# ZwwWayne/mmMOT

Hardware: NVIDIA H100
Metric: frame-pairs/sec at N=128 dets (higher is better)
Workload: dtype f32 (tensor-core engine: FP16 hi/lo split operands, fp32 accumulate)

## Files before the change

include/mmmot_b200.h:

```cpp
#ifndef MMMOT_B200_H
#define MMMOT_B200_H

#include <stddef.h>
#include <stdint.h>

#ifdef __cplusplus
extern "C" {
#endif

#define MMMOT_ABI_VERSION 2

enum {
  MMMOT_E_ARG = -1,
  MMMOT_E_WORKSPACE = -2,
  MMMOT_E_SHAPE = -3,
  MMMOT_E_RANGE = -4
};

enum { MMMOT_FUSION_A = 0, MMMOT_FUSION_B = 1, MMMOT_FUSION_C = 2 };
enum { MMMOT_AFF_MULTIPLY = 0, MMMOT_AFF_MINUS_ABS = 1, MMMOT_AFF_MINUS = 2 };
enum { MMMOT_SM_NONE = 0, MMMOT_SM_SINGLE = 1, MMMOT_SM_DUAL = 2, MMMOT_SM_DUAL_ADD = 3, MMMOT_SM_DUAL_MAX = 4 };
enum { MMMOT_END_AVG = 0, MMMOT_END_MAX = 1 };

enum mmmot_weight_id {
// ... 100 lines not shown
                     const double* det_planes, const int* det_frame, int n_dets, int* split, void* workspace,
                     size_t workspace_bytes, void* stream);
int mmmot_prep_scatter(const float* points, const int* frame_offsets, int n_frames, int stride,
                       const double* fov_planes, const double* det_planes, const int* det_frame, int n_dets,
                       const int* split, int out_channels, float* out_points, void* workspace,
                       size_t workspace_bytes, void* stream);

int mmmot_crop_resize_max_taps(void);
size_t mmmot_crop_resize_workspace(int n_det, long total_rows, int out_size, int taps);
int mmmot_crop_resize(const unsigned char* image, int img_h, int img_w, const int* boxes, const long long* row_off,
                      int n_det, long total_rows, int max_crop_h, int out_size, int taps, const float* mean_std,
                      float* out, void* workspace, size_t workspace_bytes, void* stream);

int mmmot_set_engine(int engine);

int mmmot_set_kseg(int chunks);

int mmmot_set_debug(int flags);

int mmmot_debug_linear(const float* Wt, const void* Wp, float wp_scale, const float* bias, const float* X,
                       float* Y, int M, int K, int S, int engine, void* stream);

int mmmot_debug_simt(int mode, int M, int K, const float* Wt, const float* bias, int relu, const float* X, long x_gs,
                     long x_ks, const float* sc, const float* sh, int S, int groups, const void* tile_tab, int num_tiles,
                     float* Y, long y_gs, long y_ms, void* part, void* stream);

int mmmot_debug_simt_op(int mode, int M, int K, const float* Wt, const float* bias, int relu, const float* X, long x_gs,
                        long x_ks, const float* sc, const float* sh, int n, int m, int Lf, int H, int W, int Cin, int S,
                        int groups, const void* tile_tab, int num_tiles, const float* addend, const int* seg, int ld_add,
                        float* Y, long y_gs, long y_ms, void* part, void* stream);

int mmmot_debug_gen_prefetch(int gen, int m);
int mmmot_debug_gen_staged(int gen, int m);
int mmmot_debug_gen(int gen, int M, int K, const void* Wp, float wp_scale, const float* bias, int relu, const float* src,
                    int ld_src, const float* gsc, const float* gsh, int n, int m, int Lf, int S, int groups, long x_gs,
                    long y_gs, const void* tile_tab, int num_tiles, float* Y, long y_ms, void* part, int* prefetched,
                    void* stream);

int mmmot_debug_pn_contraction(const int* det_split, const int* h_det_split, int pairs, int L, long max_tiles, void* tiles,
                               int* cnt, int* gstart, int* seg, void* ctab, long* n_tiles, const void* Wp, float wp_scale,
                               const float* bias, int M, int K, const void* Xhi, float* Y, void* part, const float* addend,
                               int ld_add, unsigned long long* segsum, const float* sc, const float* sh, void* stream);

int mmmot_debug_pn_stats(const int* det_split, const int* h_det_split, int pairs, int L, const void* Xhi, int K,
                         const float* Wt, const void* Wp, float wp_scale, const float* bias, int M, const float* addend,
                         const float* gamma, const float* beta, float* sc, float* sh, double* stats, double* mom,
                         unsigned long long* detsum, void* workspace, size_t workspace_bytes, void* stream);

int mmmot_debug_linear_planar(const void* Wp, float wp_scale, const float* bias, const void* Xhi, float* Y,
                              int M, int K, long rows, void* stream);
int mmmot_debug_conv_planar(const void* Wp, float wp_scale, const float* bias, const void* Xhi, void* Yhi,
                            int n_img, int H, int W, int C, int M, float* kseg_scratch ,
                            void* stream);

int mmmot_debug_conv_plan(int n_img, int H, int W, int C, int M, int want_pool, int use_kseg, int* plan);
int mmmot_debug_conv_layer(const void* Wp, const void* Wpx, float wp_scale, const float* bias, const void* Xhi, long x_plane,
                           int n_img, int H, int W, int C, int M, void* Yhi, long y_plane, long y_plane_pooled,
                           int* did_pool, unsigned long long* pool_sum, float* kseg_scratch, int* status, int* plan,
                           void* stream);
int mmmot_debug_vgg_conv0(const float* crops, int n_img, int H, int W, const float* wt, const float* bias, const void* Wp,
                          float wp_scale, const void* Wpx, void* Yhi, long y_plane, void* cols, int* status, int* variant,
                          void* stream);

int mmmot_debug_stage_layout(int stage, int pairs, int n, int m, size_t* offsets, int* tensor_cores);
int mmmot_debug_skip_heads(const mmmot_weights* wts, const float* pooled0, const float* pooled1, const float* pooled2,
                           const float* pooled3, int n_img, int L, float* feats, void* stream);
// ... 14 lines not shown
```

mmmot_b200/_lib.py:

```python
import ctypes
import os
import re

_HERE = os.path.dirname(os.path.abspath(__file__))
LIB_PATH = os.path.join(_HERE, "libmmmot_sm90a.so")
HEADER_PATH = os.path.join(os.path.dirname(_HERE), "include", "mmmot_b200.h")

ABI_VERSION = 2
SCORE_SIGMOID, SCORE_THRESHOLD = 1, 2
FUSION = {"A": 0, "B": 1, "C": 2}
AFFINITY = {"multiply": 0, "minus_abs": 1, "minus": 2}
SOFTMAX = {"none": 0, "single": 1, "dual": 2, "dual_add": 3, "dual_max": 4}
END_MODE = {"avg": 0, "max": 1}

W = dict(
    VGG_WT0=0, VGG_B0=13, SKIP0=26, PN_L1=66, PN_WHAT=86, PN_WHGT=87, PN_BH=88, PN_GHW=89, PN_GHB=90,
    PN_WOT=91, PN_BO=92, PN_GOW=93, PN_GOB=94,
    FU_WPT=95, FU_BP=96, FU_GPW=97, FU_GPB=98, FU_WIT=99, FU_BI=100, FU_GIW=101, FU_GIB=102,
    FU_GATE_PT=103, FU_GATE_PB=104, FU_GATE_IT=105, FU_GATE_IB=106,
    WD_W1T=107, WD_B1=108, WD_W2T=109, WD_B2=110, WD_W3=111, WD_B3=112,
    AF_W01T=113, AF_B01=114, AF_G1W=115, AF_G1B=116, AF_G0W=117, AF_G0B=118,
    AF_W2T=119, AF_B2=120, AF_G2W=121, AF_G2B=122, AF_W3T=123, AF_B3=124, AF_G3W=125, AF_G3B=126,
    AF_W4=127, AF_B4=128,
    NE_W1T=129, NE_B1=130, NE_G1W=131, NE_G1B=132, NE_W2T=133, NE_B2=134, NE_G2W=135, NE_G2B=136,
# ... 11 lines not shown
class MmmotError(RuntimeError):
    pass


_vp, _i, _l, _f, _sz = ctypes.c_void_p, ctypes.c_int, ctypes.c_long, ctypes.c_float, ctypes.c_size_t
_wp = ctypes.POINTER(Weights)

SIGNATURES = {
    "mmmot_abi_version": (_i, []),
    "mmmot_device_info": (_i, [ctypes.POINTER(_i)] * 3),
    "mmmot_launch_count": (ctypes.c_ulonglong, []),
    "mmmot_set_engine": (_i, [_i]),
    "mmmot_set_debug": (_i, [_i]),
    "mmmot_set_kseg": (_i, [_i]),
    "mmmot_debug_linear": (_i, [_vp, _vp, _f, _vp, _vp, _vp, _i, _i, _i, _i, _vp]),
    "mmmot_debug_simt": (_i, [_i, _i, _i, _vp, _vp, _i, _vp, _l, _l, _vp, _vp, _i, _i, _vp, _i, _vp, _l, _l, _vp, _vp]),
    "mmmot_debug_simt_op": (_i, [_i, _i, _i, _vp, _vp, _i, _vp, _l, _l, _vp, _vp, _i, _i, _i, _i, _i, _i, _i, _i, _vp, _i,
                                 _vp, _vp, _i, _vp, _l, _l, _vp, _vp]),
    "mmmot_debug_linear_planar": (_i, [_vp, _f, _vp, _vp, _vp, _i, _i, _l, _vp]),
    "mmmot_debug_conv_planar": (_i, [_vp, _f, _vp, _vp, _vp, _i, _i, _i, _i, _i, _vp, _vp]),
    "mmmot_debug_conv_plan": (_i, [_i, _i, _i, _i, _i, _i, _i, ctypes.POINTER(_i)]),
    "mmmot_debug_conv_layer": (_i, [_vp, _vp, _f, _vp, _vp, _l, _i, _i, _i, _i, _i, _vp, _l, _l, ctypes.POINTER(_i), _vp, _vp,
                                    _vp, ctypes.POINTER(_i), _vp]),
    "mmmot_debug_vgg_conv0": (_i, [_vp, _i, _i, _i, _vp, _vp, _vp, _f, _vp, _vp, _l, _vp, _vp, ctypes.POINTER(_i), _vp]),
    "mmmot_timing_enable": (_i, [_i]),
    "mmmot_timing_tag_count": (_i, []),
    "mmmot_timing_tag_name": (ctypes.c_char_p, [_i]),
    "mmmot_timing_collect_tags": (_i, [ctypes.POINTER(ctypes.c_double)] * 3 + [ctypes.POINTER(ctypes.c_long)]),
    "mmmot_status_reset": (_i, [_vp, _vp]),
    "mmmot_status_check": (_i, [_vp, _vp]),
    "mmmot_fetch_pinned_i32": (_i, [_vp, _vp, _l, _vp]),
    "mmmot_debug_gen_prefetch": (_i, [_i, _i]),
    "mmmot_debug_gen_staged": (_i, [_i, _i]),
    "mmmot_debug_gen": (_i, [_i, _i, _i, _vp, _f, _vp, _i, _vp, _i, _vp, _vp, _i, _i, _i, _i, _i, _l, _l, _vp, _i, _vp, _l, _vp,
                             ctypes.POINTER(_i), _vp]),
    "mmmot_debug_pn_contraction": (_i, [_vp, _vp, _i, _i, _l, _vp, _vp, _vp, _vp, _vp, ctypes.POINTER(_l), _vp, _f, _vp, _i, _i,
                                        _vp, _vp, _vp, _vp, _i, _vp, _vp, _vp, _vp]),
    "mmmot_debug_pn_stats": (_i, [_vp, _vp, _i, _i, _vp, _i, _vp, _vp, _f, _vp, _i, _vp, _vp, _vp, _vp, _vp, _vp, _vp, _vp, _vp,
                                  _sz, _vp]),
    "mmmot_debug_stage_layout": (_i, [_i, _i, _i, _i, ctypes.POINTER(_sz), ctypes.POINTER(_i)]),
    "mmmot_debug_skip_heads": (_i, [_wp, _vp, _vp, _vp, _vp, _i, _i, _vp, _vp]),
    "mmmot_timing_collect": (_i, [ctypes.POINTER(ctypes.c_double), ctypes.POINTER(ctypes.c_double), ctypes.POINTER(ctypes.c_long)]),
    "mmmot_appearance_workspace": (_sz, [_i, _i, _i]),
    "mmmot_appearance_fwd": (_i, [_wp, _vp, _i, _i, _i, _i, _vp, _vp, _sz, _vp]),
    "mmmot_appearance_train_workspace": (_sz, [_i, _i, _i]),
    "mmmot_appearance_train_fwd": (_i, [_wp, _vp, _i, _i, _i, _i, _vp, _vp, _vp, _vp, _vp, _sz, _vp]),
    "mmmot_pointnet_train_workspace": (_sz, [_i, _i, _l]),
    "mmmot_pointnet_train_fwd": (_i, [_wp, _vp, _vp, _vp, _i, _i, _vp, _vp, _vp, _sz, _vp]),
    "mmmot_w_det_train_workspace": (_sz, [_i]),
    "mmmot_w_det_train_fwd": (_i, [_wp, _i, _vp, _vp, _vp, _vp, _sz, _vp]),
    "mmmot_pointnet_workspace": (_sz, [_i, _i, _l]),
    "mmmot_pointnet_fwd": (_i, [_wp, _vp, _vp, _vp, _i, _i, _vp, _vp, _sz, _vp]),
    "mmmot_fusion_det_workspace": (_sz, [_i, _i]),
    "mmmot_fusion_det_fwd": (_i, [_wp, _i, _i, _f, _i, _i, _vp, _vp, _vp, _sz, _vp]),
    "mmmot_affinity_workspace": (_sz, [_i, _i, _i]),
    "mmmot_affinity_fwd": (_i, [_wp, _i, _i, _i, _i, _i, _i, _vp, _vp, _vp, _vp, _vp, _sz, _vp]),
    "mmmot_crop_workspace": (_sz, [_i, _i]),
    "mmmot_crop_count": (_i, [_vp, _i, _i, _vp, _i, _i, _vp, _vp, _sz, _vp]),
    "mmmot_crop_scatter": (_i, [_vp, _i, _i, _vp, _i, _i, _vp, _i, _vp, _vp, _sz, _vp]),
    "mmmot_prep_workspace": (_sz, [_i, _i, _i]),
    "mmmot_prep_count": (_i, [_vp, _vp, _i, _i, _vp, _vp, _vp, _i, _vp, _vp, _sz, _vp]),
    "mmmot_prep_scatter": (_i, [_vp, _vp, _i, _i, _vp, _vp, _vp, _i, _vp, _i, _vp, _vp, _sz, _vp]),
    "mmmot_crop_resize_max_taps": (_i, []),
    "mmmot_crop_resize_workspace": (_sz, [_i, _l, _i, _i]),
    "mmmot_crop_resize": (_i, [_vp, _i, _i, _vp, _vp, _i, _l, _i, _i, _i, _vp, _vp, _vp, _sz, _vp]),
    "mmmot_lp_workspace": (_sz, [_i, _i, _i]),
# ... 40 lines not shown
```

mmmot_b200/csrc/api.cu:

```cuda
#include <algorithm>
#include <atomic>

#include "common.cuh"

static std::atomic<unsigned long long> g_launches{0};

void mm_count_launch() { g_launches.fetch_add(1, std::memory_order_relaxed); }

extern "C" unsigned long long mmmot_launch_count(void) { return g_launches.load(); }

extern "C" int mmmot_abi_version(void) { return MMMOT_ABI_VERSION; }

int mm_sm_count(int* sms) {
  static std::atomic<int> cache[64];
  int dev = 0;
  MM_CUDA(cudaGetDevice(&dev));
  int v = cache[dev & 63].load(std::memory_order_relaxed);
  if (!v) {
    MM_CUDA(cudaDeviceGetAttribute(&v, cudaDevAttrMultiProcessorCount, dev));
    cache[dev & 63].store(v, std::memory_order_relaxed);
  }
  *sms = v;
  return 0;
}
// ... 202 lines not shown
  p.Wt = Wt; p.ldw = M; p.bias = bias; p.M = M; p.K = K; p.relu = relu;
  if (tile_tab) {
    p.tile_tab = (const int4*)tile_tab; p.num_tiles = num_tiles;
  } else {
    p.S = S; p.tiles_per_group = mm_cdiv(S, 128); p.num_tiles = p.tiles_per_group * groups;
  }
  p.X = X; p.x_gs = x_gs; p.x_ks = x_ks; p.sc = sc; p.sh = sh;
  p.n = n; p.m = m; p.Lf = Lf;
  p.H = H; p.W = W; p.Cin = Cin;
  p.addend = addend; p.seg = seg; p.ld_add = ld_add;
  p.Y = Y; p.y_gs = y_gs; p.y_ms = y_ms;
  p.part = (double2*)part;
  cudaStream_t st = (cudaStream_t)stream;
  switch (mode) {
    case XM_DIRECT: return gemm_simt_launch<XM_DIRECT>(p, st);
    case XM_NORM_RELU: return gemm_simt_launch<XM_NORM_RELU>(p, st);
    case XM_PAIR_MUL: return gemm_simt_launch<XM_PAIR_MUL>(p, st);
    case XM_PAIR_ABS: return gemm_simt_launch<XM_PAIR_ABS>(p, st);
    case XM_PAIR_SUB: return gemm_simt_launch<XM_PAIR_SUB>(p, st);
    default: return gemm_simt_launch<XM_CONV3>(p, st);
  }
}

extern "C" int mmmot_debug_gen_prefetch(int gen, int m) {
  if (gen < gen::GEN_PAIR_MUL || gen > gen::GEN_COPY) return MMMOT_E_ARG;
  return gen_prefetch(gen, m, mm_debug_flags()) ? 1 : 0;
}

extern "C" int mmmot_debug_gen_staged(int gen, int m) {
  if (gen < gen::GEN_PAIR_MUL || gen > gen::GEN_COPY) return MMMOT_E_ARG;
  return gen_staged(gen, m, mm_debug_flags()) ? 1 : 0;
}

extern "C" int mmmot_debug_gen(int gen, int M, int K, const void* Wp, float wp_scale, const float* bias, int relu,
                               const float* src, int ld_src, const float* gsc, const float* gsh, int n, int m, int Lf, int S,
                               int groups, long x_gs, long y_gs, const void* tile_tab, int num_tiles, float* Y, long y_ms,
                               void* part, int* prefetched, void* stream) {
  if (M <= 0 || K <= 0) return MMMOT_E_ARG;
  GemmP p = gemm_defaults();
  p.bias = bias; p.M = M; p.K = K; p.relu = relu;
  if (tile_tab) {
    if (num_tiles <= 0) return MMMOT_E_ARG;
    p.tile_tab = (const int4*)tile_tab; p.num_tiles = num_tiles;
  } else {
    if (S <= 0 || groups <= 0) return MMMOT_E_ARG;
    p.S = S; p.tiles_per_group = mm_cdiv(S, tc::BN); p.num_tiles = p.tiles_per_group * groups;
    p.x_gs = x_gs; p.y_gs = y_gs;
  }
  p.Y = Y; p.y_ms = y_ms;
  p.part = (double2*)part;
  const uint4* w = (const uint4*)Wp;
  cudaStream_t st = (cudaStream_t)stream;
  switch (gen) {
    case gen::GEN_PAIR_MUL: return gemm_gen_launch<gen::GEN_PAIR_MUL>(p, w, wp_scale, src, ld_src, gsc, gsh, n, m, Lf, st, prefetched);
    case gen::GEN_PAIR_ABS: return gemm_gen_launch<gen::GEN_PAIR_ABS>(p, w, wp_scale, src, ld_src, gsc, gsh, n, m, Lf, st, prefetched);
    case gen::GEN_PAIR_SUB: return gemm_gen_launch<gen::GEN_PAIR_SUB>(p, w, wp_scale, src, ld_src, gsc, gsh, n, m, Lf, st, prefetched);
    case gen::GEN_NORM: return gemm_gen_launch<gen::GEN_NORM>(p, w, wp_scale, src, ld_src, gsc, gsh, n, m, Lf, st, prefetched);
    case gen::GEN_COPY: return gemm_gen_launch<gen::GEN_COPY>(p, w, wp_scale, src, ld_src, gsc, gsh, n, m, Lf, st, prefetched);
    default: return MMMOT_E_ARG;
  }
}

extern "C" int mmmot_debug_linear_planar(const void* Wp, float wp_scale, const float* bias, const void* Xhi,
                                         float* Y, int M, int K, long rows, void* stream) {
  if (!Wp || !Xhi || !Y || M <= 0 || K <= 0 || rows <= 0) return MMMOT_E_ARG;
  GemmP p = gemm_defaults();
// ... 53 lines not shown
```

mmmot_b200/csrc/gemm_gen.cuh:

```cuda
#pragma once
#include "gemm_tma.cuh"

namespace gen {

using namespace tc;

enum { GEN_PAIR_MUL = 0, GEN_PAIR_ABS = 1, GEN_PAIR_SUB = 2, GEN_NORM = 3, GEN_COPY = 4 };

constexpr int G_EPI_WARPS = 8, G_PROD_WARP0 = 8, G_PROD_WARPS = 8;
constexpr int G_THREADS = (G_PROD_WARP0 + G_PROD_WARPS) * 32;
constexpr int G_CONS_REGS = 176, G_PROD_REGS = 80;
static_assert(256 * G_CONS_REGS + 256 * G_PROD_REGS <= launch_regs(G_THREADS) * G_THREADS, "register split exceeds the CTA's pool");
constexpr int G_DET_BYTES = 128 * BK * 4, G_OBJ_BYTES = 2 * BK * 4;
static_assert(G_DET_BYTES == A_SUB && A_SUB % 1024 == 0, "the detection box fills the stage's free 1024-aligned slot");
constexpr int G_SRC_AHEAD = STAGES - 1;
constexpr size_t G_SMEM_BYTES = (size_t)STAGES * STAGE_BYTES + 1024 + 256 + STAGES * G_OBJ_BYTES;
constexpr int G_MAX_K = 512;
__host__ __device__ constexpr bool staged(int GEN, bool PAIRED) { return PAIRED && GEN <= GEN_PAIR_SUB; }

struct GenP {
  TcP t;
  const float* src;
  int ld_src;
  const float* gsc;
  const float* gsh;
  int n, m, Lf;
};

__device__ __forceinline__ void lds128(uint32_t addr, float4& v) {
  asm volatile("ld.shared.v4.f32 {%0, %1, %2, %3}, [%4];" : "=f"(v.x), "=f"(v.y), "=f"(v.z), "=f"(v.w) : "r"(addr));
}
__device__ __forceinline__ void ld_global_256(const float* p, float (&v)[8]) {
  asm volatile("ld.global.nc.v4.f32 {%0, %1, %2, %3}, [%8];\n\tld.global.nc.v4.f32 {%4, %5, %6, %7}, [%8+16];"
               : "=f"(v[0]), "=f"(v[1]), "=f"(v[2]), "=f"(v[3]), "=f"(v[4]), "=f"(v[5]), "=f"(v[6]), "=f"(v[7])
               : "l"(p));
}

template <int GEN, bool PAIRED>
static __global__ void __launch_bounds__(G_THREADS, 1)
gemm_gen_kernel(const GenP P, const __grid_constant__ CUtensorMap map_det, const __grid_constant__ CUtensorMap map_obj) {
  const GemmP& p = P.t.g;
  extern __shared__ uint8_t smem_raw[];
  __shared__ __align__(16) float s_gsc[GEN == GEN_NORM ? G_MAX_K : 4], s_gsh[GEN == GEN_NORM ? G_MAX_K : 4];
  const uint32_t raw = smem_u32(smem_raw);
  const uint32_t base = (raw + 1023u) & ~1023u;
  uint8_t* sm = smem_raw + (base - raw);
  const uint32_t bar0 = base + STAGES * STAGE_BYTES;
  auto full_bar = [&](int s) { return bar0 + 8u * s; };
  auto empty_bar = [&](int s) { return bar0 + 8u * (STAGES + s); };
  const uint32_t free_bar = bar0 + 8u * (2 * STAGES);
  auto src_full = [&](int s) { return bar0 + 8u * (2 * STAGES + 1 + s); };
  auto src_empty = [&](int s) { return bar0 + 8u * (3 * STAGES + 1 + s); };
  const uint32_t obj0 = bar0 + 256;
  float* img = reinterpret_cast<float*>(sm);

  const int tid = threadIdx.x, warp = tid >> 5, lane = tid & 31;
  const int mgroups = P.t.m_tiles;
  const long total_tiles = (long)p.num_tiles * mgroups;
  const int KC = P.t.k_chunks;

  if (tid == 0) {
    for (int s = 0; s < STAGES; s++) {
      mbar_init(full_bar(s), 1 + G_PROD_WARPS);
      mbar_init(empty_bar(s), G_EPI_WARPS);
      if (staged(GEN, PAIRED)) {
        mbar_init(src_full(s), 1);
        mbar_init(src_empty(s), G_PROD_WARPS);
      }
    }
    mbar_init(free_bar, G_EPI_WARPS);
    asm volatile("fence.mbarrier_init.release.cluster;" ::: "memory");
  }
  __syncthreads();

  auto tile_cols = [&](int nt, int& g, int& c0, int& len) {
    if (p.tile_tab) { const int4 tt = p.tile_tab[nt]; g = tt.x; c0 = tt.y; len = tt.z; return; }
    g = nt / p.tiles_per_group;
    c0 = (nt - g * p.tiles_per_group) * BN;
    len = min(BN, p.S - c0);
  };

  if (warp < G_EPI_WARPS) {
    asm volatile("setmaxnreg.inc.sync.aligned.u32 %0;" ::"n"(G_CONS_REGS));
    const int q = warp & 3, half = warp >> 2;
    uint32_t it = 0;
    float acc[2][64];
    auto clear_acc = [&]() {
#pragma unroll
      for (int mb = 0; mb < 2; mb++)
#pragma unroll
        for (int i = 0; i < 64; i++) acc[mb][i] = 0.f;
    };
    if (!staged(GEN, PAIRED)) clear_acc();
    for (long t = blockIdx.x; t < total_tiles; t += gridDim.x) {
      const int mg = (int)(t % mgroups);
      const int nt = (int)(t / mgroups);
      int g, c0, len;
      tile_cols(nt, g, c0, len);
      if (staged(GEN, PAIRED)) clear_acc();
      for (int kc = 0; kc < KC; kc++, it++) {
        const int s = it % STAGES;
        mbar_wait(full_bar(s), (it / STAGES) & 1);
        const uint32_t sa = base + s * STAGE_BYTES, sb = sa + 2 * A_SUB + half * (128 / 8) * 128;
        if (!(P.t.dbg & 8)) {
          wgmma_fence();
#pragma unroll
          for (int ks = 0; ks < 2; ks++) {
            const uint64_t b_hi = smem_desc(sb + ks * 2 * B_LBO, B_LBO, SBO);
            const uint64_t b_lo = smem_desc(sb + B_HALF + ks * 2 * B_LBO, B_LBO, SBO);
#pragma unroll
            for (int mb = 0; mb < 2; mb++) {
              const uint32_t a = sa + mb * 8 * SBO + ks * 2 * A_LBO;
              const uint64_t a_hi = smem_desc(a, A_LBO, SBO), a_lo = smem_desc(a + A_HALF, A_LBO, SBO);
              wgmma_n128(acc[mb], a_hi, b_hi, (kc | ks) ? 1u : 0u);
              wgmma_n128(acc[mb], a_hi, b_lo, 1u);
              wgmma_n128(acc[mb], a_lo, b_hi, 1u);
            }
          }
          wgmma_commit();
        }
        wgmma_wait<1>();
        if (kc > 0) { __syncwarp(); if (lane == 0) mbar_arrive(empty_bar((it - 1) % STAGES)); }
      }
      wgmma_wait<0>();
      fence_acc(acc[0]);
      fence_acc(acc[1]);
      __syncwarp();
      if (lane == 0) mbar_arrive(empty_bar((it - 1) % STAGES));
      bar_sync(7, G_EPI_WARPS * 32);
      acc_dump(acc[0], img, BN, 0, half * 128);
      acc_dump(acc[1], img, BN, 64, half * 128);
      bar_sync(7, G_EPI_WARPS * 32);
      {
        const int co = mg * 128 + q * 32 + lane;
        const bool rowok = co < p.M;
        const float bv = (rowok && p.bias) ? __ldg(p.bias + co) : 0.f;
        double f1 = 0.0, f2 = 0.0;
        float* dst = p.Y + ((long)g * p.y_gs + c0 + half * 128) * p.y_ms + co;
#pragma unroll 1
        for (int cc = 0; cc < 4; cc++) {
          const int col0 = half * 128 + cc * 32;
          if (col0 >= len) break;
          uint32_t v[32];
          acc_ld32(img, BN, q * 32 + lane, col0, v);
          if (P.t.dbg & 1) continue;
          float s1 = 0.f, s2 = 0.f, pv = 0.f;
          if (col0 + 32 <= len) {
            if (p.relu) epi_fast<true>(v, P.t.out_scale, bv, pv, s1, s2);
            else epi_fast<false>(v, P.t.out_scale, bv, pv, s1, s2);
          } else {
            float t = 0.f;
#pragma unroll
            for (int j = 0; j < 32; j++) {
              float x = fmaf(__uint_as_float(v[j]), P.t.out_scale, bv);
              if (p.relu) x = fmaxf(x, 0.f);
              v[j] = __float_as_uint(x);
              if (col0 + j < len) t += x;
            }
            pv = t / (float)(len - col0);
#pragma unroll
            for (int j = 0; j < 32; j++)
              if (col0 + j < len) { const float d = __uint_as_float(v[j]) - pv; s1 += d; s2 = fmaf(d, d, s2); }
          }
          stat_fold(f1, f2, min(32, len - col0), pv, s1, s2);
          if (p.Y && rowok) {
            float* d = dst + (long)cc * 32 * p.y_ms;
            if (col0 + 32 <= len) {
#pragma unroll
              for (int j = 0; j < 32; j++) { *d = __uint_as_float(v[j]); d += p.y_ms; }
            } else {
#pragma unroll
              for (int j = 0; j < 32; j++)
                if (col0 + j < len) d[(long)j * p.y_ms] = __uint_as_float(v[j]);
            }
          }
        }
        if (p.part && rowok) p.part[((long)nt * 2 + half) * p.M + co] = make_double2(f1, f2);
      }
      fence_async_smem();
      __syncwarp();
      if (lane == 0) mbar_arrive(free_bar);
    }
  } else {
    asm volatile("setmaxnreg.dec.sync.aligned.u32 %0;" ::"n"(G_PROD_REGS));
    constexpr bool STAGED = staged(GEN, PAIRED);
    constexpr bool PREFETCH = PAIRED && !STAGED;
    constexpr bool ROWS = GEN == GEN_NORM || GEN == GEN_COPY;
    constexpr int NA = (ROWS || !PAIRED) ? 4 : 2;
    constexpr int NB = ROWS ? 0 : (PAIRED ? 2 : 4);
    const int pt = tid - G_PROD_WARP0 * 32;
    const int kg = (pt >> 3) & 3;
    const int cb = (pt & 7) + 8 * (pt >> 5);
    const uint32_t off0 = (uint32_t)kg * B_LBO + (uint32_t)(cb >> 3) * 128u + (uint32_t)(cb & 7) * 16u;
    uint32_t it = 0, wcount = 0;
    int g_staged = -1;
    struct Raw { float a[NA][8]; float b[NB ? NB : 1][8]; };
    for (long t = blockIdx.x; t < total_tiles; t += gridDim.x) {
      const int mg = (int)(t % mgroups);
      const int nt = (int)(t / mgroups);
      int g, c0, len;
      tile_cols(nt, g, c0, len);
      if (wcount > 0) mbar_wait(free_bar, (wcount - 1) & 1);
      wcount++;
      unsigned okmask = 0;
      const float* tbase = ROWS ? P.src + ((long)g * p.x_gs + c0) * P.ld_src : P.src + (long)g * P.Lf * p.K;
      int oa[NA], ob[NB ? NB : 1];
#pragma unroll
      for (int r = 0; r < 4; r++) {
        const int col = cb + 64 * r;
        if (col < len) okmask |= 1u << r;
        const int cc = min(col, len - 1);
        if (ROWS) {
          oa[r] = cc * P.ld_src + kg * 8;
        } else {
          const int s = c0 + cc;
          const int i = s / P.m, j = s - i * P.m;
          if (!PAIRED) {
            oa[r] = i * p.K + kg * 8;
            ob[r] = (P.n + j) * p.K + kg * 8;
          } else {
            if (!(r & 1)) oa[r >> 1] = i * p.K + kg * 8;
            if (r < 2) ob[r] = (P.n + j) * p.K + kg * 8;
          }
        }
      }
      if (GEN == GEN_NORM && g != g_staged) {
        asm volatile("bar.sync 1, %0;" ::"n"(G_PROD_WARPS * 32) : "memory");
        for (int k = pt; k < p.K; k += G_PROD_WARPS * 32) {
          s_gsc[k] = __ldg(P.gsc + (long)g * p.K + k);
          s_gsh[k] = __ldg(P.gsh + (long)g * p.K + k);
        }
        asm volatile("bar.sync 1, %0;" ::"n"(G_PROD_WARPS * 32) : "memory");
        g_staged = g;
      }
      auto load = [&](Raw& R, int kc) {
        if (P.t.dbg & 4) return;
#pragma unroll
        for (int r = 0; r < NA; r++) ld_global_256(tbase + oa[r] + kc * BK, R.a[r]);
#pragma unroll
        for (int r = 0; r < NB; r++) ld_global_256(tbase + ob[r] + kc * BK, R.b[r]);
      };
      auto emit = [&](const Raw& R, int kc) {
        const int s = it % STAGES;
        mbar_wait(empty_bar(s), ((it / STAGES) & 1) ^ 1u);
        if (pt == 0) {
          if (P.t.dbg & 2) {
            mbar_arrive(full_bar(s));
          } else {
            mbar_expect_tx(full_bar(s), A_SUB);
            bulk_g2s(base + s * STAGE_BYTES, reinterpret_cast<const uint8_t*>(P.t.Wp) + ((size_t)kc * P.t.m_tiles + mg) * A_SUB,
                     A_SUB, full_bar(s));
          }
        }
        uint8_t* bh = sm + s * STAGE_BYTES + 2 * A_SUB + off0;
        if (!(P.t.dbg & 4)) {
          const uint32_t sca = smem_u32(s_gsc + kc * BK + kg * 8), sha = smem_u32(s_gsh + kc * BK + kg * 8);
          float4 sc0, sc1, sh0, sh1;
#pragma unroll
          for (int r = 0; r < 4; r++) {
            float x[8];
            if (GEN == GEN_NORM) {
              const float(&y)[8] = R.a[r];
              if (!PAIRED ? r == 0 : !(r & 1)) { lds128(sca, sc0); lds128(sca + 16, sc1); lds128(sha, sh0); lds128(sha + 16, sh1); }
              x[0] = fmaxf(fmaf(y[0], sc0.x, sh0.x), 0.f); x[1] = fmaxf(fmaf(y[1], sc0.y, sh0.y), 0.f);
              x[2] = fmaxf(fmaf(y[2], sc0.z, sh0.z), 0.f); x[3] = fmaxf(fmaf(y[3], sc0.w, sh0.w), 0.f);
              x[4] = fmaxf(fmaf(y[4], sc1.x, sh1.x), 0.f); x[5] = fmaxf(fmaf(y[5], sc1.y, sh1.y), 0.f);
              x[6] = fmaxf(fmaf(y[6], sc1.z, sh1.z), 0.f); x[7] = fmaxf(fmaf(y[7], sc1.w, sh1.w), 0.f);
            } else if (GEN == GEN_COPY) {
#pragma unroll
              for (int e = 0; e < 8; e++) x[e] = R.a[r][e];
            } else {
              const float(&av)[8] = R.a[PAIRED ? (r >> 1) : r];
              const float(&bv)[8] = R.b[NB ? (PAIRED ? (r & 1) : r) : 0];
#pragma unroll
              for (int e = 0; e < 8; e++) {
                if (GEN == GEN_PAIR_MUL) x[e] = av[e] * bv[e];
                else if (GEN == GEN_PAIR_ABS) x[e] = fabsf(av[e] - bv[e]) * 0.5f;
                else x[e] = (av[e] - bv[e]) * 0.5f;
              }
            }
            uint32_t h[4], l[4];
#pragma unroll
            for (int q = 0; q < 4; q++) split_f16x2(x[2 * q], x[2 * q + 1], h[q], l[q]);
            if (!((okmask >> r) & 1u)) { h[0] = h[1] = h[2] = h[3] = 0u; l[0] = l[1] = l[2] = l[3] = 0u; }
            *reinterpret_cast<uint4*>(bh + r * 1024) = make_uint4(h[0], h[1], h[2], h[3]);
            *reinterpret_cast<uint4*>(bh + B_HALF + r * 1024) = make_uint4(l[0], l[1], l[2], l[3]);
          }
        }
        fence_async_smem();
        __syncwarp();
        if (lane == 0) mbar_arrive(full_bar(s));
        it++;
      };
      if (STAGED) {
        const bool gen_ops = !(P.t.dbg & 4);
        const int row_det = g * P.Lf + P.n, row_obj = g * P.Lf + c0 / P.m;
        auto issue = [&](uint32_t pos, int kc) {
          const int s = pos % STAGES;
          mbar_wait(src_empty(s), ((pos / STAGES) & 1) ^ 1u);
          mbar_expect_tx(src_full(s), G_DET_BYTES + G_OBJ_BYTES);
          tma::tma_load_2d(base + s * STAGE_BYTES + A_SUB, &map_det, kc * BK, row_det, src_full(s));
          tma::tma_load_2d(obj0 + s * G_OBJ_BYTES, &map_obj, kc * BK, row_obj, src_full(s));
        };
        if (pt == 0 && gen_ops)
          for (int kc = 0; kc < KC && kc < G_SRC_AHEAD; kc++) issue(it + kc, kc);
        const uint32_t u0 = (uint32_t)(((2 * kg) ^ (cb & 7)) * 16), u1 = (uint32_t)(((2 * kg + 1) ^ (cb & 7)) * 16);
        for (int kc = 0; kc < KC; kc++) {
          const int s = it % STAGES;
          mbar_wait(empty_bar(s), ((it / STAGES) & 1) ^ 1u);
          if (pt == 0) {
            if (P.t.dbg & 2) {
              mbar_arrive(full_bar(s));
            } else {
              mbar_expect_tx(full_bar(s), A_SUB);
              bulk_g2s(base + s * STAGE_BYTES, reinterpret_cast<const uint8_t*>(P.t.Wp) + ((size_t)kc * P.t.m_tiles + mg) * A_SUB,
                       A_SUB, full_bar(s));
            }
          }
          if (gen_ops) {
            uint8_t* bh = sm + s * STAGE_BYTES + 2 * A_SUB + off0;
            const uint32_t db = base + s * STAGE_BYTES + A_SUB + (uint32_t)cb * 128u, ob = obj0 + s * G_OBJ_BYTES + kg * 32;
            mbar_wait(src_full(s), (it / STAGES) & 1);
            float4 d[2][2];
            lds128(db + u0, d[0][0]); lds128(db + u1, d[0][1]);
            lds128(db + 64 * 128 + u0, d[1][0]); lds128(db + 64 * 128 + u1, d[1][1]);
#pragma unroll
            for (int a = 0; a < 2; a++) {
              float4 o[2];
              lds128(ob + a * BK * 4, o[0]); lds128(ob + a * BK * 4 + 16, o[1]);
              const float av[8] = {o[0].x, o[0].y, o[0].z, o[0].w, o[1].x, o[1].y, o[1].z, o[1].w};
#pragma unroll
              for (int b = 0; b < 2; b++) {
                const int r = 2 * a + b;
                const float bv[8] = {d[b][0].x, d[b][0].y, d[b][0].z, d[b][0].w, d[b][1].x, d[b][1].y, d[b][1].z, d[b][1].w};
                float x[8];
#pragma unroll
                for (int e = 0; e < 8; e++) {
                  if (GEN == GEN_PAIR_MUL) x[e] = av[e] * bv[e];
                  else if (GEN == GEN_PAIR_ABS) x[e] = fabsf(av[e] - bv[e]) * 0.5f;
                  else x[e] = (av[e] - bv[e]) * 0.5f;
                }
                uint32_t h[4], l[4];
#pragma unroll
                for (int q = 0; q < 4; q++) split_f16x2(x[2 * q], x[2 * q + 1], h[q], l[q]);
                if (!((okmask >> r) & 1u)) { h[0] = h[1] = h[2] = h[3] = 0u; l[0] = l[1] = l[2] = l[3] = 0u; }
                *reinterpret_cast<uint4*>(bh + r * 1024) = make_uint4(h[0], h[1], h[2], h[3]);
                *reinterpret_cast<uint4*>(bh + B_HALF + r * 1024) = make_uint4(l[0], l[1], l[2], l[3]);
              }
            }
            __syncwarp();
            if (lane == 0) mbar_arrive(src_empty(s));
          }
          fence_async_smem();
          __syncwarp();
          if (lane == 0) mbar_arrive(full_bar(s));
          if (pt == 0 && gen_ops && kc + G_SRC_AHEAD < KC) issue(it + G_SRC_AHEAD, kc + G_SRC_AHEAD);
          it++;
        }
      } else if (PREFETCH) {
        Raw R0, R1;
        load(R0, 0);
        for (int kc = 0; kc < KC; kc += 2) {
          if (kc + 1 < KC) load(R1, kc + 1);
          emit(R0, kc);
          if (kc + 1 < KC) {
            if (kc + 2 < KC) load(R0, kc + 2);
            emit(R1, kc + 1);
          }
        }
      } else {
        for (int kc = 0; kc < KC; kc++) {
          Raw R;
          load(R, kc);
          emit(R, kc);
        }
      }
    }
  }
}

}

template <int GEN, bool PAIRED>
static int gemm_gen_launch_t(const GemmP& g, const uint4* Wp, float out_scale, const float* src, int ld_src,
                           const float* gsc, const float* gsh, int n, int m, int Lf, cudaStream_t st) {
  if (!Wp || !src || g.num_tiles <= 0 || g.K % tc::BK) return MMMOT_E_ARG;
  if (g.tile_tab && ((GEN != gen::GEN_NORM && GEN != gen::GEN_COPY) || g.x_gs || g.y_gs)) return MMMOT_E_ARG;
  if (GEN == gen::GEN_NORM && (g.K > gen::G_MAX_K || !gsc || !gsh)) return MMMOT_E_ARG;
  if ((GEN == gen::GEN_NORM || GEN == gen::GEN_COPY) && (ld_src < g.K || (ld_src & 7))) return MMMOT_E_ARG;
  int sms = 0;
  MM_TRY(mm_sm_count(&sms));
  static std::atomic<unsigned long long> attr{0};
  MM_TRY(mm_ensure_smem(gen::gemm_gen_kernel<GEN, PAIRED>, gen::G_SMEM_BYTES, attr));
  gen::GenP P;
  memset(&P, 0, sizeof(P));
  P.t.g = g;
  P.t.Wp = Wp;
  P.t.m_tiles = (g.M + 127) / 128;
  P.t.k_chunks = g.K / tc::BK;
  P.t.out_scale = out_scale;
  P.t.out_mode = tc::OUT_CL;
  P.t.dbg = mm_debug_flags();
  P.src = src; P.ld_src = ld_src; P.gsc = gsc; P.gsh = gsh;
  P.n = n; P.m = m; P.Lf = Lf;
  alignas(64) CUtensorMap map_det, map_obj;
  memset(&map_det, 0, sizeof(map_det));
  memset(&map_obj, 0, sizeof(map_obj));
  if (gen::staged(GEN, PAIRED)) {
    if (m != 128 || Lf != n + m || g.tile_tab || g.tiles_per_group <= 0) return MMMOT_E_ARG;
    const long rows = (long)(g.num_tiles / g.tiles_per_group) * Lf;
    MM_TRY(tma::make_map_2d_f32(&map_det, src, rows, g.K, 128, CU_TENSOR_MAP_SWIZZLE_128B));
    MM_TRY(tma::make_map_2d_f32(&map_obj, src, rows, g.K, 2, CU_TENSOR_MAP_SWIZZLE_NONE));
  }
  const long total = (long)g.num_tiles * P.t.m_tiles;
  const int grid = (int)(total < sms ? total : sms);
  gen::gemm_gen_kernel<GEN, PAIRED><<<grid, gen::G_THREADS, gen::G_SMEM_BYTES, st>>>(P, map_det, map_obj);
  MM_LAUNCH_CHECK();
  return 0;
}

static inline bool gen_prefetch(int GEN, int m, int dbg) {
  if (dbg & 1024) return false;
  if (GEN == gen::GEN_NORM) return (dbg & 4096) != 0;
  if (GEN == gen::GEN_COPY) return true;
  return m == 128;
}

static inline bool gen_staged(int GEN, int m, int dbg) {
  return GEN <= gen::GEN_PAIR_SUB && gen_prefetch(GEN, m, dbg);
}

template <int GEN>
static int gemm_gen_launch(const GemmP& g, const uint4* Wp, float out_scale, const float* src, int ld_src,
                           const float* gsc, const float* gsh, int n, int m, int Lf, cudaStream_t st,
                           int* prefetched = nullptr) {
  const bool pipe = gen_prefetch(GEN, m, mm_debug_flags());
  if (prefetched) *prefetched = pipe ? 1 : 0;
  if (pipe) return gemm_gen_launch_t<GEN, true>(g, Wp, out_scale, src, ld_src, gsc, gsh, n, m, Lf, st);
  return gemm_gen_launch_t<GEN, false>(g, Wp, out_scale, src, ld_src, gsc, gsh, n, m, Lf, st);
}
```

Baseline: 197.6.

## Add tall 256x128 tile shape to generated-operand GEMM when M tiles are even

Adds a TALL template variant of the generated-operand wgmma GEMM. Each work unit covers 256 output rows by 128 columns instead of 128 by 256, and the two consumer warpgroups split rows instead of columns. The generated B operand is built once per 128 columns and shared across twice as many weight rows, which halves the on-the-fly operand generation per output element. It is chosen automatically when the number of 128-row M tiles is even and the staged TMA path is not in use. In exchange, weight loads per stage double, there are more work units, and empty half-tiles need zeroed partial statistics.

```diff
diff --git a/include/mmmot_b200.h b/include/mmmot_b200.h
--- a/include/mmmot_b200.h
+++ b/include/mmmot_b200.h
@@ -156,6 +156,7 @@
 
 int mmmot_debug_gen_prefetch(int gen, int m);
 int mmmot_debug_gen_staged(int gen, int m);
+int mmmot_debug_gen_tall(int gen, int M, int m);
 int mmmot_debug_gen(int gen, int M, int K, const void* Wp, float wp_scale, const float* bias, int relu, const float* src,
                     int ld_src, const float* gsc, const float* gsh, int n, int m, int Lf, int S, int groups, long x_gs,
                     long y_gs, const void* tile_tab, int num_tiles, float* Y, long y_ms, void* part, int* prefetched,
diff --git a/mmmot_b200/_lib.py b/mmmot_b200/_lib.py
--- a/mmmot_b200/_lib.py
+++ b/mmmot_b200/_lib.py
@@ -67,6 +67,7 @@
     "mmmot_fetch_pinned_i32": (_i, [_vp, _vp, _l, _vp]),
     "mmmot_debug_gen_prefetch": (_i, [_i, _i]),
     "mmmot_debug_gen_staged": (_i, [_i, _i]),
+    "mmmot_debug_gen_tall": (_i, [_i, _i, _i]),
     "mmmot_debug_gen": (_i, [_i, _i, _i, _vp, _f, _vp, _i, _vp, _i, _vp, _vp, _i, _i, _i, _i, _i, _l, _l, _vp, _i, _vp, _l, _vp,
                              ctypes.POINTER(_i), _vp]),
     "mmmot_debug_pn_contraction": (_i, [_vp, _vp, _i, _i, _l, _vp, _vp, _vp, _vp, _vp, ctypes.POINTER(_l), _vp, _f, _vp, _i, _i,
diff --git a/mmmot_b200/csrc/api.cu b/mmmot_b200/csrc/api.cu
--- a/mmmot_b200/csrc/api.cu
+++ b/mmmot_b200/csrc/api.cu
@@ -258,6 +258,11 @@
   return gen_staged(gen, m, mm_debug_flags()) ? 1 : 0;
 }
 
+extern "C" int mmmot_debug_gen_tall(int gen, int M, int m) {
+  if (gen < gen::GEN_PAIR_MUL || gen > gen::GEN_COPY || M <= 0) return MMMOT_E_ARG;
+  return gen_tall(gen, M, m, mm_debug_flags()) ? 1 : 0;
+}
+
 extern "C" int mmmot_debug_gen(int gen, int M, int K, const void* Wp, float wp_scale, const float* bias, int relu,
                                const float* src, int ld_src, const float* gsc, const float* gsh, int n, int m, int Lf, int S,
                                int groups, long x_gs, long y_gs, const void* tile_tab, int num_tiles, float* Y, long y_ms,
diff --git a/mmmot_b200/csrc/gemm_gen.cuh b/mmmot_b200/csrc/gemm_gen.cuh
--- a/mmmot_b200/csrc/gemm_gen.cuh
+++ b/mmmot_b200/csrc/gemm_gen.cuh
@@ -12,7 +12,7 @@
 constexpr int G_CONS_REGS = 176, G_PROD_REGS = 80;
 static_assert(256 * G_CONS_REGS + 256 * G_PROD_REGS <= launch_regs(G_THREADS) * G_THREADS, "register split exceeds the CTA's pool");
 constexpr int G_DET_BYTES = 128 * BK * 4, G_OBJ_BYTES = 2 * BK * 4;
-static_assert(G_DET_BYTES == A_SUB && A_SUB % 1024 == 0, "the detection box fills the stage's free 1024-aligned slot");
+static_assert(G_DET_BYTES == A_SUB && A_SUB % 1024 == 0, "the detection box fills a 1024-aligned 16 KB slot of the stage");
 constexpr int G_SRC_AHEAD = STAGES - 1;
 constexpr size_t G_SMEM_BYTES = (size_t)STAGES * STAGE_BYTES + 1024 + 256 + STAGES * G_OBJ_BYTES;
 constexpr int G_MAX_K = 512;
@@ -36,10 +36,21 @@
                : "l"(p));
 }
 
-template <int GEN, bool PAIRED>
+template <int GEN, bool PAIRED, bool TALL>
 static __global__ void __launch_bounds__(G_THREADS, 1)
 gemm_gen_kernel(const GenP P, const __grid_constant__ CUtensorMap map_det, const __grid_constant__ CUtensorMap map_obj) {
   const GemmP& p = P.t.g;
+  constexpr int TM = TALL ? 256 : 128, TN = TALL ? 128 : BN;
+  constexpr int NI = TN / 64;
+  constexpr int T_A = (TM / 128) * A_SUB, T_B = 2 * A_SUB;
+  constexpr int T_BHALF = TN * BK * 2, T_BLBO = (TN / 8) * 128;
+  constexpr int T_SRC = TALL ? T_B + 2 * T_BHALF : A_SUB;
+  constexpr int T_OBJ_BYTES = (TN / 128) * BK * 4;
+  static_assert(T_A <= T_B && T_B + 2 * T_BHALF <= STAGE_BYTES, "weights and operand planes fit the stage");
+  static_assert(T_SRC % 1024 == 0 && T_SRC + G_DET_BYTES <= STAGE_BYTES && (T_SRC >= T_B + 2 * T_BHALF || (T_SRC >= T_A && T_SRC + G_DET_BYTES <= T_B)),
+                "the detection box has a 1024-aligned slot of its own in the stage");
+  static_assert(TM * TN * 4 <= 2 * STAGE_BYTES && STAGES >= 2, "the accumulator image fits the ring");
+  static_assert(T_OBJ_BYTES <= G_OBJ_BYTES, "object rows fit their area");
   extern __shared__ uint8_t smem_raw[];
   __shared__ __align__(16) float s_gsc[GEN == GEN_NORM ? G_MAX_K : 4], s_gsh[GEN == GEN_NORM ? G_MAX_K : 4];
   const uint32_t raw = smem_u32(smem_raw);
@@ -55,8 +66,8 @@
   float* img = reinterpret_cast<float*>(sm);
 
   const int tid = threadIdx.x, warp = tid >> 5, lane = tid & 31;
-  const int mgroups = P.t.m_tiles;
-  const long total_tiles = (long)p.num_tiles * mgroups;
+  const int mgroups = P.t.m_tiles / (TM / 128);
+  const long total_tiles = (long)p.num_tiles * mgroups * (BN / TN);
   const int KC = P.t.k_chunks;
 
   if (tid == 0) {
@@ -79,10 +90,20 @@
     c0 = (nt - g * p.tiles_per_group) * BN;
     len = min(BN, p.S - c0);
   };
+  auto unit = [&](long t, int& mg, int& nt, int& ch, int& g, int& c0, int& len) {
+    mg = (int)(t % mgroups);
+    const long r = t / mgroups;
+    ch = TALL ? (int)(r & 1) : 0;
+    nt = (int)(TALL ? r >> 1 : r);
+    tile_cols(nt, g, c0, len);
+    c0 += TN * ch;
+    len = min(len - TN * ch, TN);
+  };
 
   if (warp < G_EPI_WARPS) {
     asm volatile("setmaxnreg.inc.sync.aligned.u32 %0;" ::"n"(G_CONS_REGS));
     const int q = warp & 3, half = warp >> 2;
+    const int rbase = TALL ? half * 128 : 0, cbase = TALL ? 0 : half * 128;
     uint32_t it = 0;
     float acc[2][64];
     auto clear_acc = [&]() {
@@ -91,23 +112,27 @@
 #pragma unroll
         for (int i = 0; i < 64; i++) acc[mb][i] = 0.f;
     };
-    if (!staged(GEN, PAIRED)) clear_acc();
+    if (!(staged(GEN, PAIRED) || TALL)) clear_acc();
     for (long t = blockIdx.x; t < total_tiles; t += gridDim.x) {
-      const int mg = (int)(t % mgroups);
-      const int nt = (int)(t / mgroups);
-      int g, c0, len;
-      tile_cols(nt, g, c0, len);
-      if (staged(GEN, PAIRED)) clear_acc();
+      int mg, nt, ch, g, c0, len;
+      unit(t, mg, nt, ch, g, c0, len);
+      if (TALL && len <= 0) {
+        const int co = mg * TM + rbase + q * 32 + lane;
+        if (p.part && co < p.M) p.part[((long)nt * 2 + ch) * p.M + co] = make_double2(0.0, 0.0);
+        continue;
+      }
+      if (staged(GEN, PAIRED) || TALL) clear_acc();
       for (int kc = 0; kc < KC; kc++, it++) {
         const int s = it % STAGES;
         mbar_wait(full_bar(s), (it / STAGES) & 1);
-        const uint32_t sa = base + s * STAGE_BYTES, sb = sa + 2 * A_SUB + half * (128 / 8) * 128;
+        const uint32_t sa = base + s * STAGE_BYTES + (TALL ? half * A_SUB : 0);
+        const uint32_t sb = base + s * STAGE_BYTES + T_B + (TALL ? 0 : half * (128 / 8) * 128);
         if (!(P.t.dbg & 8)) {
           wgmma_fence();
 #pragma unroll
           for (int ks = 0; ks < 2; ks++) {
-            const uint64_t b_hi = smem_desc(sb + ks * 2 * B_LBO, B_LBO, SBO);
-            const uint64_t b_lo = smem_desc(sb + B_HALF + ks * 2 * B_LBO, B_LBO, SBO);
+            const uint64_t b_hi = smem_desc(sb + ks * 2 * T_BLBO, T_BLBO, SBO);
+            const uint64_t b_lo = smem_desc(sb + T_BHALF + ks * 2 * T_BLBO, T_BLBO, SBO);
 #pragma unroll
             for (int mb = 0; mb < 2; mb++) {
               const uint32_t a = sa + mb * 8 * SBO + ks * 2 * A_LBO;
@@ -128,21 +153,21 @@
       __syncwarp();
       if (lane == 0) mbar_arrive(empty_bar((it - 1) % STAGES));
       bar_sync(7, G_EPI_WARPS * 32);
-      acc_dump(acc[0], img, BN, 0, half * 128);
-      acc_dump(acc[1], img, BN, 64, half * 128);
+      acc_dump(acc[0], img, TN, rbase, cbase);
+      acc_dump(acc[1], img, TN, rbase + 64, cbase);
       bar_sync(7, G_EPI_WARPS * 32);
       {
-        const int co = mg * 128 + q * 32 + lane;
+        const int co = mg * TM + rbase + q * 32 + lane;
         const bool rowok = co < p.M;
         const float bv = (rowok && p.bias) ? __ldg(p.bias + co) : 0.f;
         double f1 = 0.0, f2 = 0.0;
-        float* dst = p.Y + ((long)g * p.y_gs + c0 + half * 128) * p.y_ms + co;
+        float* dst = p.Y + ((long)g * p.y_gs + c0 + cbase) * p.y_ms + co;
 #pragma unroll 1
         for (int cc = 0; cc < 4; cc++) {
-          const int col0 = half * 128 + cc * 32;
+          const int col0 = cbase + cc * 32;
           if (col0 >= len) break;
           uint32_t v[32];
-          acc_ld32(img, BN, q * 32 + lane, col0, v);
+          acc_ld32(img, TN, rbase + q * 32 + lane, col0, v);
           if (P.t.dbg & 1) continue;
           float s1 = 0.f, s2 = 0.f, pv = 0.f;
           if (col0 + 32 <= len) {
@@ -175,7 +200,7 @@
             }
           }
         }
-        if (p.part && rowok) p.part[((long)nt * 2 + half) * p.M + co] = make_double2(f1, f2);
+        if (p.part && rowok) p.part[((long)nt * 2 + (TALL ? ch : half)) * p.M + co] = make_double2(f1, f2);
       }
       fence_async_smem();
       __syncwarp();
@@ -186,27 +211,26 @@
     constexpr bool STAGED = staged(GEN, PAIRED);
     constexpr bool PREFETCH = PAIRED && !STAGED;
     constexpr bool ROWS = GEN == GEN_NORM || GEN == GEN_COPY;
-    constexpr int NA = (ROWS || !PAIRED) ? 4 : 2;
-    constexpr int NB = ROWS ? 0 : (PAIRED ? 2 : 4);
+    constexpr int NA = (ROWS || !PAIRED) ? NI : 2;
+    constexpr int NB = ROWS ? 0 : (PAIRED ? 2 : NI);
     const int pt = tid - G_PROD_WARP0 * 32;
     const int kg = (pt >> 3) & 3;
     const int cb = (pt & 7) + 8 * (pt >> 5);
-    const uint32_t off0 = (uint32_t)kg * B_LBO + (uint32_t)(cb >> 3) * 128u + (uint32_t)(cb & 7) * 16u;
+    const uint32_t off0 = (uint32_t)kg * T_BLBO + (uint32_t)(cb >> 3) * 128u + (uint32_t)(cb & 7) * 16u;
     uint32_t it = 0, wcount = 0;
     int g_staged = -1;
     struct Raw { float a[NA][8]; float b[NB ? NB : 1][8]; };
     for (long t = blockIdx.x; t < total_tiles; t += gridDim.x) {
-      const int mg = (int)(t % mgroups);
-      const int nt = (int)(t / mgroups);
-      int g, c0, len;
-      tile_cols(nt, g, c0, len);
+      int mg, nt, ch, g, c0, len;
+      unit(t, mg, nt, ch, g, c0, len);
+      if (TALL && len <= 0) continue;
       if (wcount > 0) mbar_wait(free_bar, (wcount - 1) & 1);
       wcount++;
       unsigned okmask = 0;
       const float* tbase = ROWS ? P.src + ((long)g * p.x_gs + c0) * P.ld_src : P.src + (long)g * P.Lf * p.K;
       int oa[NA], ob[NB ? NB : 1];
 #pragma unroll
-      for (int r = 0; r < 4; r++) {
+      for (int r = 0; r < NI; r++) {
         const int col = cb + 64 * r;
         if (col < len) okmask |= 1u << r;
         const int cc = min(col, len - 1);
@@ -233,6 +257,12 @@
         asm volatile("bar.sync 1, %0;" ::"n"(G_PROD_WARPS * 32) : "memory");
         g_staged = g;
       }
+      auto weights = [&](int s, int kc) {
+        if (P.t.dbg & 2) { mbar_arrive(full_bar(s)); return; }
+        mbar_expect_tx(full_bar(s), T_A);
+        bulk_g2s(base + s * STAGE_BYTES,
+                 reinterpret_cast<const uint8_t*>(P.t.Wp) + ((size_t)kc * P.t.m_tiles + mg * (TM / 128)) * A_SUB, T_A, full_bar(s));
+      };
       auto load = [&](Raw& R, int kc) {
         if (P.t.dbg & 4) return;
 #pragma unroll
@@ -243,21 +273,13 @@
       auto emit = [&](const Raw& R, int kc) {
         const int s = it % STAGES;
         mbar_wait(empty_bar(s), ((it / STAGES) & 1) ^ 1u);
-        if (pt == 0) {
-          if (P.t.dbg & 2) {
-            mbar_arrive(full_bar(s));
-          } else {
-            mbar_expect_tx(full_bar(s), A_SUB);
-            bulk_g2s(base + s * STAGE_BYTES, reinterpret_cast<const uint8_t*>(P.t.Wp) + ((size_t)kc * P.t.m_tiles + mg) * A_SUB,
-                     A_SUB, full_bar(s));
-          }
-        }
-        uint8_t* bh = sm + s * STAGE_BYTES + 2 * A_SUB + off0;
+        if (pt == 0) weights(s, kc);
+        uint8_t* bh = sm + s * STAGE_BYTES + T_B + off0;
         if (!(P.t.dbg & 4)) {
           const uint32_t sca = smem_u32(s_gsc + kc * BK + kg * 8), sha = smem_u32(s_gsh + kc * BK + kg * 8);
           float4 sc0, sc1, sh0, sh1;
 #pragma unroll
-          for (int r = 0; r < 4; r++) {
+          for (int r = 0; r < NI; r++) {
             float x[8];
             if (GEN == GEN_NORM) {
               const float(&y)[8] = R.a[r];
@@ -284,7 +306,7 @@
             for (int q = 0; q < 4; q++) split_f16x2(x[2 * q], x[2 * q + 1], h[q], l[q]);
             if (!((okmask >> r) & 1u)) { h[0] = h[1] = h[2] = h[3] = 0u; l[0] = l[1] = l[2] = l[3] = 0u; }
             *reinterpret_cast<uint4*>(bh + r * 1024) = make_uint4(h[0], h[1], h[2], h[3]);
-            *reinterpret_cast<uint4*>(bh + B_HALF + r * 1024) = make_uint4(l[0], l[1], l[2], l[3]);
+            *reinterpret_cast<uint4*>(bh + T_BHALF + r * 1024) = make_uint4(l[0], l[1], l[2], l[3]);
           }
         }
         fence_async_smem();
@@ -298,8 +320,8 @@
         auto issue = [&](uint32_t pos, int kc) {
           const int s = pos % STAGES;
           mbar_wait(src_empty(s), ((pos / STAGES) & 1) ^ 1u);
-          mbar_expect_tx(src_full(s), G_DET_BYTES + G_OBJ_BYTES);
-          tma::tma_load_2d(base + s * STAGE_BYTES + A_SUB, &map_det, kc * BK, row_det, src_full(s));
+          mbar_expect_tx(src_full(s), G_DET_BYTES + T_OBJ_BYTES);
+          tma::tma_load_2d(base + s * STAGE_BYTES + T_SRC, &map_det, kc * BK, row_det, src_full(s));
           tma::tma_load_2d(obj0 + s * G_OBJ_BYTES, &map_obj, kc * BK, row_obj, src_full(s));
         };
         if (pt == 0 && gen_ops)
@@ -308,24 +330,16 @@
         for (int kc = 0; kc < KC; kc++) {
           const int s = it % STAGES;
           mbar_wait(empty_bar(s), ((it / STAGES) & 1) ^ 1u);
-          if (pt == 0) {
-            if (P.t.dbg & 2) {
-              mbar_arrive(full_bar(s));
-            } else {
-              mbar_expect_tx(full_bar(s), A_SUB);
-              bulk_g2s(base + s * STAGE_BYTES, reinterpret_cast<const uint8_t*>(P.t.Wp) + ((size_t)kc * P.t.m_tiles + mg) * A_SUB,
-                       A_SUB, full_bar(s));
-            }
-          }
+          if (pt == 0) weights(s, kc);
           if (gen_ops) {
-            uint8_t* bh = sm + s * STAGE_BYTES + 2 * A_SUB + off0;
-            const uint32_t db = base + s * STAGE_BYTES + A_SUB + (uint32_t)cb * 128u, ob = obj0 + s * G_OBJ_BYTES + kg * 32;
+            uint8_t* bh = sm + s * STAGE_BYTES + T_B + off0;
+            const uint32_t db = base + s * STAGE_BYTES + T_SRC + (uint32_t)cb * 128u, ob = obj0 + s * G_OBJ_BYTES + kg * 32;
             mbar_wait(src_full(s), (it / STAGES) & 1);
             float4 d[2][2];
             lds128(db + u0, d[0][0]); lds128(db + u1, d[0][1]);
             lds128(db + 64 * 128 + u0, d[1][0]); lds128(db + 64 * 128 + u1, d[1][1]);
 #pragma unroll
-            for (int a = 0; a < 2; a++) {
+            for (int a = 0; a < TN / 128; a++) {
               float4 o[2];
               lds128(ob + a * BK * 4, o[0]); lds128(ob + a * BK * 4 + 16, o[1]);
               const float av[8] = {o[0].x, o[0].y, o[0].z, o[0].w, o[1].x, o[1].y, o[1].z, o[1].w};
@@ -345,7 +359,7 @@
                 for (int q = 0; q < 4; q++) split_f16x2(x[2 * q], x[2 * q + 1], h[q], l[q]);
                 if (!((okmask >> r) & 1u)) { h[0] = h[1] = h[2] = h[3] = 0u; l[0] = l[1] = l[2] = l[3] = 0u; }
                 *reinterpret_cast<uint4*>(bh + r * 1024) = make_uint4(h[0], h[1], h[2], h[3]);
-                *reinterpret_cast<uint4*>(bh + B_HALF + r * 1024) = make_uint4(l[0], l[1], l[2], l[3]);
+                *reinterpret_cast<uint4*>(bh + T_BHALF + r * 1024) = make_uint4(l[0], l[1], l[2], l[3]);
               }
             }
             __syncwarp();
@@ -381,7 +395,7 @@
 
 }
 
-template <int GEN, bool PAIRED>
+template <int GEN, bool PAIRED, bool TALL>
 static int gemm_gen_launch_t(const GemmP& g, const uint4* Wp, float out_scale, const float* src, int ld_src,
                            const float* gsc, const float* gsh, int n, int m, int Lf, cudaStream_t st) {
   if (!Wp || !src || g.num_tiles <= 0 || g.K % tc::BK) return MMMOT_E_ARG;
@@ -391,12 +405,13 @@
   int sms = 0;
   MM_TRY(mm_sm_count(&sms));
   static std::atomic<unsigned long long> attr{0};
-  MM_TRY(mm_ensure_smem(gen::gemm_gen_kernel<GEN, PAIRED>, gen::G_SMEM_BYTES, attr));
+  MM_TRY(mm_ensure_smem(gen::gemm_gen_kernel<GEN, PAIRED, TALL>, gen::G_SMEM_BYTES, attr));
   gen::GenP P;
   memset(&P, 0, sizeof(P));
   P.t.g = g;
   P.t.Wp = Wp;
   P.t.m_tiles = (g.M + 127) / 128;
+  if (TALL && ((P.t.m_tiles & 1) || gen::staged(GEN, PAIRED))) return MMMOT_E_ARG;
   P.t.k_chunks = g.K / tc::BK;
   P.t.out_scale = out_scale;
   P.t.out_mode = tc::OUT_CL;
@@ -410,11 +425,11 @@
     if (m != 128 || Lf != n + m || g.tile_tab || g.tiles_per_group <= 0) return MMMOT_E_ARG;
     const long rows = (long)(g.num_tiles / g.tiles_per_group) * Lf;
     MM_TRY(tma::make_map_2d_f32(&map_det, src, rows, g.K, 128, CU_TENSOR_MAP_SWIZZLE_128B));
-    MM_TRY(tma::make_map_2d_f32(&map_obj, src, rows, g.K, 2, CU_TENSOR_MAP_SWIZZLE_NONE));
+    MM_TRY(tma::make_map_2d_f32(&map_obj, src, rows, g.K, TALL ? 1 : 2, CU_TENSOR_MAP_SWIZZLE_NONE));
   }
   const long total = (long)g.num_tiles * P.t.m_tiles;
   const int grid = (int)(total < sms ? total : sms);
-  gen::gemm_gen_kernel<GEN, PAIRED><<<grid, gen::G_THREADS, gen::G_SMEM_BYTES, st>>>(P, map_det, map_obj);
+  gen::gemm_gen_kernel<GEN, PAIRED, TALL><<<grid, gen::G_THREADS, gen::G_SMEM_BYTES, st>>>(P, map_det, map_obj);
   MM_LAUNCH_CHECK();
   return 0;
 }
@@ -428,6 +443,10 @@
 
 static inline bool gen_staged(int GEN, int m, int dbg) {
   return GEN <= gen::GEN_PAIR_SUB && gen_prefetch(GEN, m, dbg);
+}
+
+static inline bool gen_tall(int GEN, int M, int m, int dbg) {
+  return !(dbg & 2048) && ((M + 127) / 128) % 2 == 0 && !gen_staged(GEN, m, dbg);
 }
 
 template <int GEN>
@@ -436,6 +455,9 @@
                            int* prefetched = nullptr) {
   const bool pipe = gen_prefetch(GEN, m, mm_debug_flags());
   if (prefetched) *prefetched = pipe ? 1 : 0;
-  if (pipe) return gemm_gen_launch_t<GEN, true>(g, Wp, out_scale, src, ld_src, gsc, gsh, n, m, Lf, st);
-  return gemm_gen_launch_t<GEN, false>(g, Wp, out_scale, src, ld_src, gsc, gsh, n, m, Lf, st);
-}
+  const bool tall = gen_tall(GEN, g.M, m, mm_debug_flags());
+  if (pipe && tall) return gemm_gen_launch_t<GEN, true, true>(g, Wp, out_scale, src, ld_src, gsc, gsh, n, m, Lf, st);
+  if (pipe) return gemm_gen_launch_t<GEN, true, false>(g, Wp, out_scale, src, ld_src, gsc, gsh, n, m, Lf, st);
+  if (tall) return gemm_gen_launch_t<GEN, false, true>(g, Wp, out_scale, src, ld_src, gsc, gsh, n, m, Lf, st);
+  return gemm_gen_launch_t<GEN, false, false>(g, Wp, out_scale, src, ld_src, gsc, gsh, n, m, Lf, st);
+}
```

New measurement: 202.1, median of 6. 1.02x the previous value.
